# phylo42/IPK

Hardware: AMD Instinct MI355X
Metric: scored phylo-k-mers/sec (higher is better)
Workload: dtype f32

## Files before the change

ipk_amd/csrc/ipkgpu.hip:

```cpp
#include <cstring>
#include <hip/hip_runtime.h>
#include <rocprim/rocprim.hpp>

#include <algorithm>
#include <cmath>
#include <cstdarg>
#include <cstdio>
#include <cstring>
#include <new>
#include <string>
#include <type_traits>
#include <unordered_map>
#include <memory>
#include <vector>

#include "../../include/ipkgpu.h"
#include "dcla_device.hpp"
#include "kernels_score.hpp"
#include "kernels_quad.hpp"
#include "kernels_compact.hpp"
#include "kernels_keymajor.hpp"
#include "kernels_reduce_pipe.hpp"
#include "kernels_filter.hpp"
#include "kernels_dbfile.hpp"
// ... 53 lines not shown
struct ipkgpu_ctx {
    int device = 0;
    ipkgpu_comm* comm = nullptr;
    hipStream_t stream = nullptr;
    std::string err;
    int64_t workspace_bytes = 0;
    int64_t opt_variant = 0;
    int64_t opt_flags = 0;
    int64_t opt_kmc_pass = 0;
    int64_t opt_prefix_mats = 0;
    int64_t opt_wg_chunks2 = 0;
    int64_t opt_rounds = 0;
    int64_t opt_pool_limit = 0;
    int64_t opt_pool_chunks = 0;
    DevBuf table, best, ovfq, counts, offsets, goff, idx, branch, scan_sums, scan_boff, tmp_a, tmp_b, tmp_c;
    DevBuf pool, desc, gbcnt, gboff, gbcur, clist, gm, tile_next;
    DevBuf ptrs;
    DevBuf sp_bits, sp_pops, sp_rank, sp_c16;
    void* h_spill[2] = {nullptr, nullptr}; hipEvent_t ev_spill[2] = {nullptr, nullptr}; size_t h_spill_cap = 0;
    size_t held = 0, held_peak = 0;
    int64_t budget = 0;
    size_t refused_need = 0;
    DevBuf mask;
    bool mask_valid = false;
    uint64_t mask_words = 0;
    bool table_compressed = false;
    DevBuf rank, vaddr, ucnt, qpack, xstart, pcounts;
    DevBuf seq, pvals, pvaddr, mrank, cursnap;
    DevBuf cvals, coff, croom;
    bool comp_own_vals = false;
    std::vector<uint32_t> h_branch;
    uint32_t comp_nb = 0, comp_stride = 0, comp_tbl = 0;
    double pairs_per_window = 0;
    double acc_main_ms = 0, acc_reduce_ms = 0;
    double acc_count_ms = 0, acc_write_ms = 0, acc_km_ms = 0;
    const char* main_kernel = "";
    std::vector<std::pair<void*, size_t>> free_blocks;
    std::unordered_map<void*, size_t> live_blocks;
    size_t cached_bytes = 0, cache_limit = 0;
    void* small = nullptr;
    void* h_up = nullptr; size_t h_up_cap = 0; hipEvent_t up_done = nullptr; bool up_pending = false;
    unsigned long long emitted_host = 0; bool emitted_fetched = false;
    uint32_t* h_rb = nullptr;
    EventPool events;
    bool spec_skip_wait = false;
    uint64_t pool_want_min = 0;
    struct Pending {
        bool active = false;
        std::unique_ptr<Stopwatch> sw; int ev_a = -1, ev_b = -1, ev_c = -1, ev_d = -1;
        uint64_t cap = 0, max_chunks = 0, windows = 0; uint32_t gb = 0; bool pool_ovf_ok = false, use_quad = false;
    } pend;
    uint64_t last_entries = 0; uint32_t last_gb = 0;
    double t_write_total = 0, t_write_device = 0, t_write_file = 0;
    int num_cu = 256;
};

struct ipkgpu_result {
    ipkgpu_ctx* ctx = nullptr;
    std::vector<uint32_t> group_ids;
    std::vector<uint64_t> offsets;
    uint64_t emitted = 0;
    uint32_t* d_keys = nullptr;
    float* d_scores = nullptr;
    uint32_t* d_positions = nullptr;
    size_t cap = 0;
// ... 187 lines not shown
        *got = ctx->free_blocks[best].second;
        ctx->live_blocks[*out] = *got;
        ctx->cached_bytes -= *got;
        ctx->free_blocks.erase(ctx->free_blocks.begin() + best);
        return hipSuccess;
    }
    const hipError_t e = ctx_alloc(ctx, out, want_bytes);
    if (e == hipSuccess) *got = ctx->live_blocks[*out];
    return e;
}

static std::vector<DevBuf*> all_workspaces(ipkgpu_ctx* ctx)
{
    return {&ctx->table, &ctx->best, &ctx->ovfq, &ctx->counts, &ctx->offsets, &ctx->goff, &ctx->idx,
            &ctx->branch, &ctx->scan_sums, &ctx->scan_boff, &ctx->tmp_a, &ctx->tmp_b, &ctx->tmp_c,
            &ctx->pool, &ctx->desc, &ctx->gbcnt, &ctx->gboff, &ctx->gbcur, &ctx->clist, &ctx->gm, &ctx->tile_next, &ctx->mask,
            &ctx->rank, &ctx->vaddr, &ctx->ucnt, &ctx->qpack, &ctx->xstart, &ctx->pcounts, &ctx->ptrs,
            &ctx->cvals, &ctx->coff, &ctx->croom, &ctx->seq, &ctx->pvals, &ctx->pvaddr, &ctx->mrank, &ctx->cursnap,
            &ctx->sp_bits, &ctx->sp_pops, &ctx->sp_rank, &ctx->sp_c16};
}

extern "C" {

uint32_t ipkgpu_bits_per_symbol(uint32_t sigma) { return sigma == 4 ? 2u : sigma == 20 ? 5u : 0u; }
uint32_t ipkgpu_max_k(uint32_t sigma) { return sigma == 4 ? 14u : sigma == 20 ? 6u : 0u; }
uint32_t ipkgpu_max_k_keyrange(uint32_t sigma) { return sigma == 4 ? 16u : ipkgpu_max_k(sigma); }
size_t ipkgpu_kmer_batch(uint32_t key, size_t n_ranges) { return n_ranges ? key % n_ranges : 0; }

float ipkgpu_log_threshold(float omega, uint32_t sigma, uint32_t k)
{
    return log10f(powf(omega / (float)sigma, (float)k));
// ... 188 lines not shown
        constexpr int CAP = fast_cap<SIGMA, K>();
        constexpr uint32_t T = ipow(SIGMA, K);
        constexpr uint32_t NB = (T + TBL - 1) / TBL;
        constexpr int SNW = stream_nw<SIGMA, K>(), STW = stream_tw<SIGMA, K>();
        constexpr size_t lds = TileGeo<SIGMA, K, STW>::HEAD_BYTES + (size_t)SNW * stream_wave_scratch<SIGMA, K, CAP>() * 8 + (size_t)SNW * 2 * NB * SUB * 4;
        static_assert(lds <= 160 * 1024, "stream pass-1 LDS budget");
        auto kern = score_stream_kernel<SIGMA, K, CAP, STW, SNW, TBL>;
        if (lds > 64 * 1024)
            HIP_TRY(ctx, hipFuncSetAttribute(reinterpret_cast<const void*>(kern), hipFuncAttributeMaxDynamicSharedMemorySize, (int)lds));
        hipLaunchKernelGGL(kern, dim3(n_wg), dim3(SNW * 64), lds, ctx->stream, sp);
        HIP_TRY(ctx, hipGetLastError());
        return IPKGPU_OK;
    }
}

template <int SIGMA, int K>
int launch_stream_overflow(ipkgpu_ctx* ctx, const StreamParams& sp)
{
    constexpr uint32_t TBL = stream_tbl<SIGMA, K>();
    if constexpr (TBL == 0 || ipow(SIGMA, K - K / 2) <= (uint32_t)fast_cap<SIGMA, K>()) {
        (void)ctx; (void)sp;
        return IPKGPU_OK;
    } else {
        constexpr uint32_t NB = (uint32_t)((ipow(SIGMA, K) + TBL - 1) / TBL);
        constexpr size_t lds = TileGeo<SIGMA, K, 1>::HEAD_BYTES + (size_t)wave_scratch_entries<SIGMA, K, big_capf<SIGMA, K>()>() * 8 +
                               (size_t)OVF_NW * 2 * NB * SUB * 4;
        static_assert(lds + 64 <= 160 * 1024, "big-list (stream) LDS budget");
        auto kern = score_overflow_stream_kernel<SIGMA, K, TBL>;
        if (lds > 64 * 1024)
            HIP_TRY(ctx, hipFuncSetAttribute(reinterpret_cast<const void*>(kern), hipFuncAttributeMaxDynamicSharedMemorySize, (int)lds));
        const uint32_t per_cu = (uint32_t)std::max<size_t>(1, std::min<size_t>(32 / OVF_NW, (160 * 1024) / (lds + 64)));
        hipLaunchKernelGGL(kern, dim3(ctx->num_cu * per_cu), dim3(OVF_NW * 64), lds, ctx->stream, sp);
        HIP_TRY(ctx, hipGetLastError());
        return IPKGPU_OK;
    }
}

#ifndef IPK_RPIPE_DEFAULT
#define IPK_RPIPE_DEFAULT 1
#endif
#ifndef IPK_RPIPE_D
#define IPK_RPIPE_D 2
#endif
template <int SIGMA, int K>
int launch_stream_pass2(ipkgpu_ctx* ctx, uint32_t n_gb, uint64_t T, uint32_t* table, bool compress)
{
    constexpr uint32_t TBL = stream_tbl<SIGMA, K>();
// ... 274 lines not shown
{
    CompTable ct;
    ct.mask = ctx->mask.as<uint32_t>(); ct.rank = ctx->rank.as<uint32_t>(); ct.vaddr = ctx->vaddr.as<uint64_t>();
    ct.pool = ctx->comp_own_vals ? ctx->cvals.as<uint2>() : ctx->pool.as<uint2>();
    ct.off = ctx->comp_own_vals ? ctx->coff.as<uint64_t>() : ctx->gboff.as<uint64_t>(); ct.mask_words = ctx->mask_words;
    ct.NB = ctx->comp_nb; ct.stride = ctx->comp_stride; ct.TBL = ctx->comp_tbl;
    return ct;
}

}

namespace {

constexpr int IPKGPU_RETRY_SMALLER = 100;
constexpr int IPKGPU_RETRY_AGAIN = 101;
#ifndef IPK_OVF_POOL_RATIO
#define IPK_OVF_POOL_RATIO 500
#endif

enum class PassKind { tiles, stream, quad, xp };
struct Pass {
    PassKind kind = PassKind::tiles;
    bool positions = false;
    bool compress = false;
    bool seq = false;
    double slot_bytes() const { return positions ? 8.0 : kind == PassKind::xp && compress ? 0.3125 : 4.0; }
};

Pass choose_pass(int64_t variant, uint32_t sigma, uint32_t lead, bool positions, bool km_positions, const Geometry& g)
{
    Pass ps;
    ps.positions = positions;
    if (positions) return ps;
// ... 217 lines not shown
    pd.active = false;
    std::unique_ptr<Stopwatch> sw(pd.sw.release());
    const uint32_t n_ovf = ctx->h_rb[SMALL_OVF_COUNT / 4], pool_exhausted = ctx->h_rb[SMALL_POOL_OVF / 4];
    if (pool_exhausted) {
        if (pd.cap >= pd.max_chunks) {
            ctx->pool_want_min = 0;
            if (pd.gb > 1) return IPKGPU_RETRY_SMALLER;
            return fail(ctx, IPKGPU_ERR_NOMEM, "the pair pool of ONE branch group is exhausted at the device-memory limit");
        }
        ctx->pool_want_min = pd.cap * 2;
        return IPKGPU_RETRY_AGAIN;
    }
    ctx->pool_want_min = 0;
    memcpy(&ctx->emitted_host, ctx->h_rb + SMALL_EMITTED / 4, 8);
    ctx->emitted_fetched = true;
    ctx->spec_skip_wait = !(n_ovf > 0 && (uint64_t)n_ovf * IPK_OVF_POOL_RATIO >= pd.windows && pd.pool_ovf_ok);
    if (sw) { ctx->acc_main_ms += sw->ms(pd.ev_a, pd.ev_b); ctx->acc_reduce_ms += sw->ms(pd.ev_c, pd.ev_d); }
    return IPKGPU_OK;
}

int arm_capped(ipkgpu_ctx* ctx, uint32_t sigma, uint32_t k, ScoreParams& p)
{
    const bool capped_lists = sigma == 4 && k >= 13;
    p.big_ovf = capped_lists ? small_at(ctx, SMALL_BIG_OVF) : nullptr;
    if (capped_lists) HIP_TRY(ctx, hipMemsetAsync(p.big_ovf, 0, 4, ctx->stream));
    return IPKGPU_OK;
}

int check_capped(ipkgpu_ctx* ctx, uint32_t k, const ScoreParams& p)
{
    if (!p.big_ovf) return IPKGPU_OK;
// ... 162 lines not shown
    const uint64_t max_wg = std::max<uint64_t>(slots, expected_chunks * 2 / wg_chunks2 / ((uint64_t)SNW * NBK * SUB));
#ifndef IPK_ROUNDS
#define IPK_ROUNDS 8
#endif
    const uint64_t rounds = std::max<uint64_t>(1, std::min<uint64_t>(ctx->opt_rounds > 0 ? (uint64_t)ctx->opt_rounds : (uint64_t)IPK_ROUNDS, max_wg / slots));
    uint64_t S64 = std::max<uint64_t>(1, (slots * rounds) / gb);
    uint32_t S = (uint32_t)std::max<uint64_t>(1, std::min<uint64_t>(S64, s_tiles_per_mat));
    const uint32_t n_wg = gb * S;
    const uint64_t n_waves = (uint64_t)n_wg * SNW;
    const uint64_t n_gb = (uint64_t)gb * NBK;

    const size_t free_b = mem_free_bytes(ctx);
    uint64_t max_chunks = std::min<uint64_t>(0xFFFFFFF0ull, (uint64_t)(free_b + ctx->pool.cap + ctx->desc.cap) * 9 / 10 / (CH * 8 + 8));
    if (ctx->opt_pool_limit > 0) max_chunks = std::min<uint64_t>(max_chunks, (uint64_t)ctx->opt_pool_limit / (CH * 8 + 8));
    const double ppw = ctx->pairs_per_window > 0 ? ctx->pairs_per_window : 256.0;
    const uint64_t ovf_waves = (uint64_t)ctx->num_cu * 4 * OVF_NW;
    const uint64_t slack = 2 * (n_waves + ovf_waves) * NBK * SUB + (n_waves + ovf_waves) * ALLOC_BATCH + 1024;
    uint64_t want = (uint64_t)((double)windows * ppw * 1.25 / CH) + slack;
    {
        const uint64_t have = std::min<uint64_t>(std::max<uint64_t>(ctx->pool.cap / (CH * 8), 1) - 1, ctx->desc.cap / 8);
        const uint64_t need = (uint64_t)((double)windows * ppw * 1.1 / CH) + (n_waves + ovf_waves) * (NBK * SUB + ALLOC_BATCH) + 1024;
        if (have >= need) want = have;
    }
    want = std::max<uint64_t>(want, ctx->pool_want_min);
    for (int attempt = 0; attempt < 6; ++attempt) {
        uint64_t cap = std::min<uint64_t>(want, max_chunks);
        const bool forced = attempt == 0 && ctx->opt_pool_chunks > 0 && ctx->pool_want_min == 0;
        if (forced) cap = (uint64_t)ctx->opt_pool_chunks;
        else if (cap < n_waves * NBK * SUB) {
            if (gb > 1) return IPKGPU_RETRY_SMALLER;
            return fail(ctx, IPKGPU_ERR_NOMEM, "the pair pool of ONE branch group does not fit device memory");
// ... 1 lines not shown
        RC_TRY(ensure(ctx, ctx->pool, (cap + 1) * CH * 8));
        RC_TRY(ensure(ctx, ctx->desc, cap * 8));
        if (!forced) cap = std::min<uint64_t>(ctx->pool.cap / (CH * 8) - 1, ctx->desc.cap / 8);
        RC_TRY(ensure(ctx, ctx->gbcnt, 2 * n_gb * 4));
        uint32_t* const d_gbcur = ctx->gbcnt.as<uint32_t>() + n_gb;
        RC_TRY(ensure(ctx, ctx->gboff, (n_gb + 1) * 8));
        uint32_t* d_pool_next = small_at(ctx, SMALL_POOL_NEXT);
        uint32_t* d_pool_ovf = small_at(ctx, SMALL_POOL_OVF);
        const bool pre_ok = use_quad && n_waves * NBK + 1024 <= cap && !(ctx->opt_flags & 32);
        const uint32_t pre_chunks = pre_ok ? (uint32_t)(n_waves * NBK) : 0u;
        uint32_t* d_tile_next = nullptr;
        if (use_quad && !(ctx->opt_flags & 128) && ((uint64_t)nb * s_tiles_per_mat >= 4ull * gb * S || (ctx->opt_flags & 256))) {
            RC_TRY(ensure(ctx, ctx->tile_next, (size_t)gb * 4));
            d_tile_next = ctx->tile_next.as<uint32_t>();
        }
        hipLaunchKernelGGL(small_reset_kernel, dim3((std::max<uint32_t>(gb, SMALL_XP_TOO_BIG / 4) + 255) / 256), dim3(256), 0, ctx->stream,
                           reinterpret_cast<uint32_t*>(ctx->small), pre_chunks, d_tile_next, gb, S);
        HIP_TRY(ctx, hipGetLastError());
        HIP_TRY(ctx, hipMemsetAsync(ctx->desc.p, 0, cap * 8, ctx->stream));

        StreamParams sp;
        sp.logp = logp_dev; sp.best = ctx->best.as<float>();
        sp.gm_off = ctx->gm.as<uint32_t>(); sp.gm_list = ctx->gm.as<uint32_t>() + gb + 1;
        sp.sites = pl.sites; sp.nwin = pl.nwin; sp.tiles_per_mat = s_tiles_per_mat; sp.S = S;
        sp.eps = pl.eps;
        sp.pool = ctx->pool.as<uint2>(); sp.pool_cap = (uint32_t)cap; sp.pool_next = d_pool_next;
        sp.desc = ctx->desc.as<unsigned long long>(); sp.pool_ovf = d_pool_ovf;
        sp.emitted = p.emitted; sp.ovf_queue = p.ovf_queue; sp.ovf_count = p.ovf_count; sp.mat_slot = p.mat_slot;
        sp.flags = (uint32_t)(ctx->opt_flags);
        sp.pre_chunks = pre_chunks;
        sp.tile_next = d_tile_next;
        std::unique_ptr<Stopwatch> sw_own(new Stopwatch(ctx->stream, &ctx->events));
        Stopwatch& sw = *sw_own;
        const int ev_a = sw.mark();
        RC_TRY(pass1(sp, n_wg, false));
        const int ev_b = sw.mark();
        const bool spec = ctx->spec_skip_wait && !s_compress && !(ctx->opt_flags & 64);
        uint32_t n_ovf = 0;
        uint32_t h[2] = {0, 0};
        if (!spec) {
            HIP_TRY(ctx, hipMemcpyAsync(ctx->h_rb, ctx->small, SMALL_BYTES, hipMemcpyDeviceToHost, ctx->stream));
            HIP_TRY(ctx, hipStreamSynchronize(ctx->stream));
            n_ovf = ctx->h_rb[SMALL_OVF_COUNT / 4]; h[0] = ctx->h_rb[SMALL_POOL_NEXT / 4]; h[1] = ctx->h_rb[SMALL_POOL_OVF / 4];
        }
        const bool ovf_in_pool = n_ovf > 0 && ((uint64_t)n_ovf * IPK_OVF_POOL_RATIO >= windows || s_compress) && pool_ovf_ok;
        if (ovf_in_pool) {
            RC_TRY(ensure(ctx, ctx->tmp_a, (size_t)n_ovf * 8));
            RC_TRY(ensure(ctx, ctx->tmp_b, (size_t)n_ovf * 8));
            hipLaunchKernelGGL(ovf_group_keys_kernel, dim3((n_ovf + 255) / 256), dim3(256), 0, ctx->stream,
                               p.ovf_queue, n_ovf, p.mat_slot, ctx->tmp_a.as<unsigned long long>());
            HIP_TRY(ctx, hipGetLastError());
            size_t tmp_bytes = 0;
            HIP_TRY(ctx, rocprim::radix_sort_keys(nullptr, tmp_bytes, ctx->tmp_a.as<unsigned long long>(), ctx->tmp_b.as<unsigned long long>(),
                                                  (size_t)n_ovf, 0, 64, ctx->stream));
            RC_TRY(ensure(ctx, ctx->tmp_c, tmp_bytes));
            HIP_TRY(ctx, rocprim::radix_sort_keys(ctx->tmp_c.p, tmp_bytes, ctx->tmp_a.as<unsigned long long>(), ctx->tmp_b.as<unsigned long long>(),
                                                  (size_t)n_ovf, 0, 64, ctx->stream));
            StreamParams so = sp;
            so.ovf_queue = ctx->tmp_b.as<unsigned long long>();
            if (use_quad) so.emitted = small_at<unsigned long long>(ctx, SMALL_OVF_EMITTED);
            RC_TRY(with_sigma_k(ctx, pl.sigma, pl.k, [&](auto S_, auto K_) { return launch_stream_overflow<S_, K_>(ctx, so); }));
        }
        if (ovf_in_pool) {
            HIP_TRY(ctx, hipMemcpyAsync(ctx->h_rb, ctx->small, SMALL_BYTES, hipMemcpyDeviceToHost, ctx->stream));
            HIP_TRY(ctx, hipStreamSynchronize(ctx->stream));
            h[0] = ctx->h_rb[SMALL_POOL_NEXT / 4]; h[1] = ctx->h_rb[SMALL_POOL_OVF / 4];
        }
        if (h[1] != 0) {
            if (cap >= max_chunks) {
                if (gb > 1) return IPKGPU_RETRY_SMALLER;
                return fail(ctx, IPKGPU_ERR_NOMEM, "the pair pool of ONE branch group is exhausted at the device-memory limit");
            }
            want = std::max<uint64_t>(cap * 2, want);
            continue;
        }
        const uint32_t n_used = spec ? (uint32_t)cap : (uint32_t)std::min<uint64_t>(h[0], cap);
        const uint32_t* n_used_dev = spec ? d_pool_next : nullptr;
        HIP_TRY(ctx, hipMemsetAsync(ctx->gbcnt.p, 0, 2 * n_gb * 4, ctx->stream));
// ... 22 lines not shown
            RC_TRY(ensure(ctx, ctx->vaddr, (size_t)gb * (ctx->mask_words / 2) * 8));
            RC_TRY(ensure(ctx, ctx->ucnt, n_gb * 4));
        }
        if (n_used) {
            const uint64_t n_grid = spec ? std::min<uint64_t>(n_used, expected_chunks * 2 + n_waves * NBK + 4096) : n_used;
            hipLaunchKernelGGL(chunk_scatter_kernel, dim3((uint32_t)std::min<uint64_t>((n_grid + 255) / 256, 1u << 16)), dim3(256), 0, ctx->stream,
                               ctx->desc.as<unsigned long long>(), n_used, ctx->gboff.as<uint64_t>(), d_gbcur,
                               ctx->clist.as<uint2>(), n_used_dev);
            HIP_TRY(ctx, hipGetLastError());
        }
        const int ev_c = sw.mark();
        RC_TRY(with_sigma_k(ctx, pl.sigma, pl.k, [&](auto S_, auto K_) {
            return launch_stream_pass2<S_, K_>(ctx, (uint32_t)n_gb, pl.table_size, ctx->table.as<uint32_t>(), s_compress);
        }));
        const int ev_d = sw.mark();
        if ((spec || n_ovf > 0) && !ovf_in_pool)
            RC_TRY(with_sigma_k(ctx, pl.sigma, pl.k, [&](auto S_, auto K_) { return launch_overflow<S_, K_, false>(ctx, p); }));
        if (s_compress) {
            ctx->table_compressed = true; ctx->comp_own_vals = true;
            ctx->comp_nb = NBK; ctx->comp_stride = 1; ctx->comp_tbl = TBL;
        }
        ctx->mask_valid = true;
        ctx->main_kernel = use_quad ? "score_quad_kernel" : "score_stream_kernel";
        HIP_TRY(ctx, hipMemcpyAsync(ctx->h_rb, ctx->small, SMALL_BYTES, hipMemcpyDeviceToHost, ctx->stream));
        ipkgpu_ctx::Pending& pd = ctx->pend;
        pd.sw.reset(sw_own.release());
        pd.ev_a = ev_a; pd.ev_b = ev_b; pd.ev_c = ev_c; pd.ev_d = ev_d;
        pd.cap = cap; pd.max_chunks = max_chunks; pd.windows = windows; pd.gb = gb; pd.pool_ovf_ok = pool_ovf_ok; pd.use_quad = use_quad;
        pd.active = true;
        if (defer) return IPKGPU_OK;
        HIP_TRY(ctx, hipStreamSynchronize(ctx->stream));
        const int rcf = stream_batch_check(ctx);
        if (rcf == IPKGPU_RETRY_AGAIN) { want = std::max<uint64_t>(want, ctx->pool_want_min); continue; }
        return rcf;
    }
    return fail(ctx, IPKGPU_ERR_NOMEM, "pair pool could not be sized");
}

int score_batch_finish(ipkgpu_ctx* ctx, const Plan& pl, uint32_t g0, uint32_t gb, uint64_t* emitted_acc)
{
    if (ctx->pend.active) RC_TRY(stream_batch_check(ctx));
    unsigned long long e = ctx->emitted_host;
    if (!ctx->emitted_fetched) {
// ... 1325 lines not shown
        keys += f.head.n_keys; entries += f.head.n_entries;
    }
    return IPKGPU_OK;
}

}

extern "C" {

int ipkgpu_get_option(const ipkgpu_ctx* ctx, const char* name, int64_t* value)
{
    if (!ctx || !name || !value) return IPKGPU_ERR_INVALID;
    if (!strcmp(name, "workspace_bytes")) { *value = ctx->workspace_bytes; return IPKGPU_OK; }
    if (!strcmp(name, "device_budget_bytes")) { *value = ctx->budget; return IPKGPU_OK; }
    if (!strcmp(name, "last_refused_bytes")) { *value = (int64_t)ctx->refused_need; return IPKGPU_OK; }
    return IPKGPU_ERR_INVALID;
}

int ipkgpu_mem_stats(ipkgpu_ctx* ctx, uint64_t* held, uint64_t* held_peak, int reset_peak)
{
    if (!ctx) return IPKGPU_ERR_INVALID;
    if (held) *held = ctx->held;
    if (held_peak) *held_peak = ctx->held_peak;
    if (reset_peak) ctx->held_peak = ctx->held;
    return IPKGPU_OK;
}

int ipkgpu_parts_spill(ipkgpu_ctx* ctx, ipkgpu_parts* parts, const char* dir, uint32_t piece, uint64_t* bytes_written)
{
    if (!ctx) return IPKGPU_ERR_INVALID;
// ... 198 lines not shown
```

ipk_amd/csrc/kernels_quad.hpp:

```cpp
#pragma once
#include "kernels_score.hpp"

namespace ipkgpu {

struct QuadNode { int J, H, TH, OFF; uint32_t F, CMUL; };
struct QuadStep { int H, A, B; };

template <int SIGMA, int K>
struct QuadGeo {
    using D = HalvesDD<SIGMA, K>;
    static constexpr int HL = D::HL, HR = D::HR, LA = D::LA, LB = D::LB, RA = D::RA, RB = D::RB;
    static constexpr bool OK = SIGMA == 4 && D::OK && LA >= 2 && LA <= 3 && LB >= 2 && LB <= 3 && RA >= 2 && RA <= 3 && RB >= 2 && RB <= 3;
    static constexpr uint32_t FLA = D::FLA, FLB = D::FLB, FRA = D::FRA, FRB = D::FRB;
    static constexpr uint32_t mulR = ipow(SIGMA, K - K / 2);
    static constexpr uint32_t CW = FLA + FLB + FRA + FRB;
    static constexpr int th_n(int h) { return h == 2 ? 3 : 5; }
    static constexpr int TH0 = 2, TH1 = TH0 + th_n(LA), TH2 = TH1 + th_n(LB), TH3 = TH2 + th_n(RA);
    static constexpr int TH_F = TH3 + th_n(RB);
    static constexpr int PADW = 1;
    static constexpr QuadNode node(int n)
    {
        return n == 0 ? QuadNode{0, LA, TH0, 0, FLA, 1u}
             : n == 1 ? QuadNode{LA, LB, TH1, (int)FLA, FLB, mulR}
             : n == 2 ? QuadNode{HL, RA, TH2, (int)(FLA + FLB), FRA, 1u}
// ... 430 lines not shown
                    const bool p0 = v0 && c0, p1 = v1 && c1;
                    const uint64_t h0 = ballot64(v0) & ballot64(c0), h1 = ballot64(v1) & ballot64(c1);
                    if (p0) lp[mbcnt(h0)] = make_uint2(a0.x * (Q::FLB * mulR) + b0.x, __float_as_uint(s0));
                    if (p1) rp[mbcnt(h1)] = make_uint2(a1.x * Q::FRB + b1.x, __float_as_uint(s1));
                    nL = (uint32_t)__popcll(h0); nR = (uint32_t)__popcll(h1);
                } else {
                    if (!keep_l)
                        nL = (uint32_t)__builtin_amdgcn_readfirstlane((int)join_to_list(la + ia, min(sla, nla - ia), lb, nlb, eps_l, Q::FLB * mulR, lp, CAPL));
                    if constexpr (SLICE) {
                        if (nL == LIST_OVERFLOW) { sla = SAFE_L; continue; }
                    }
                    nR = nL == LIST_OVERFLOW || nL == 0 ? nL : (uint32_t)__builtin_amdgcn_readfirstlane((int)join_to_list(ra + ir, min(sra, nra - ir), rb, nrb, eps_r, Q::FRB, rp, CAPR));
                    if constexpr (SLICE) {
                        if (nR == LIST_OVERFLOW) { sra = SAFE_R; keep_l = true; continue; }
                    } else if (nL == LIST_OVERFLOW || nR == LIST_OVERFLOW) {
                        if (lane == 0) {
                            const uint32_t qi = atomicAdd(p.ovf_count, 1u);
                            p.ovf_queue[qi] = ((unsigned long long)mat << 32) | (unsigned long long)(t0 + w);
                        }
                        __builtin_amdgcn_wave_barrier();
                        break;
                    }
                }
                if (nL != 0 && nR != 0) {
                wave_lds_sync();
                if (p.flags & 4u) emitted += nL + nR;
                else
                if constexpr (ROWLANE) {
                    constexpr uint32_t CB = 64;
                    static_assert(CB <= CH, "row-per-lane join: a run must fit a chunk");
                    for (uint32_t ib = 0; ib < nL; ib += 64) {
                        const uint2 a = lp[ib + lane];
                        const bool rv = ib + lane < nL;
                        const float ay = rv ? __uint_as_float(a.y) : -__builtin_inff();
// ... 178 lines not shown
```

ipk_amd/csrc/kernels_score.hpp:

```cpp
#pragma once
#include <type_traits>
#include "dcla_device.hpp"

namespace ipkgpu {


template <int SIGMA, int M>
__global__ __launch_bounds__(256) void prefix_max_kernel(const float* __restrict__ logp, uint32_t n_mats, uint32_t sites,
                                                         float* __restrict__ best)
{
    constexpr int CH = 2048 / M;
    constexpr int ROW = CH + 4;
    static_assert(M == 1 || M == 2 || M == 4 || M == 8, "matrices per workgroup");
    __shared__ __align__(16) float cmbuf[2][M][ROW];
    const uint32_t mat0 = blockIdx.x * M;
    const uint32_t mv = min((uint32_t)M, n_mats - mat0);
    const bool chain = threadIdx.x < mv;
    const uint32_t my = mat0 + (chain ? threadIdx.x : 0u);
    float* b = best + (size_t)my * (sites + 1);
    if (chain) b[0] = 0.0f;
    float carry = 0.0f;
    auto maxima = [&](uint32_t c0, float (*cmw)[ROW], uint32_t t0, uint32_t nt) {
        const uint32_t n = min((uint32_t)CH, sites - c0);
        for (uint32_t mm = 0; mm < mv; ++mm) {
// ... 311 lines not shown
    uint32_t sites, nwin, tiles_per_mat, S;
    float eps;
    uint2* pool;
    uint32_t pool_cap;
    uint32_t* pool_next;
    unsigned long long* desc;
    uint32_t* pool_ovf;
    unsigned long long* emitted;
    unsigned long long* ovf_queue;
    uint32_t* ovf_count;
    const uint32_t* mat_slot;
    uint32_t flags;
    uint32_t pre_chunks;
    uint32_t* tile_next = nullptr;
    uint32_t* big_ovf = nullptr;
};

__device__ __constant__ uint32_t RCP16[65] = {
    0, 65536, 32768, 21846, 16384, 13108, 10923, 9363, 8192, 7282, 6554, 5958, 5462, 5042, 4682, 4370, 4096,
    3856, 3641, 3450, 3277, 3121, 2979, 2850, 2731, 2622, 2521, 2428, 2341, 2260, 2185, 2115, 2048,
    1986, 1928, 1873, 1821, 1772, 1725, 1681, 1639, 1599, 1561, 1525, 1490, 1457, 1425, 1395, 1366,
    1338, 1311, 1286, 1261, 1237, 1214, 1192, 1171, 1150, 1130, 1111, 1093, 1075, 1058, 1041, 1024};

template <int SIGMA, int K>
struct HalvesDD {
    static constexpr int HL = K / 2, HR = K - K / 2;
    static constexpr int LA = HL / 2, LB = HL - LA, RA = HR / 2, RB = HR - RA;
    static constexpr bool OK = ipow(SIGMA, HL) > 64 && ipow(SIGMA, LB) <= 64 && ipow(SIGMA, RB) <= 64;
    static constexpr uint32_t FLA = ipow(SIGMA, LA), FLB = ipow(SIGMA, LB), FRA = ipow(SIGMA, RA), FRB = ipow(SIGMA, RB);
};
template <int SIGMA, int K, int CAP>
// ... 175 lines not shown
            const uint32_t n4 = ncol * (SIGMA / 4);
            for (uint32_t i = threadIdx.x; i < n4; i += NW * 64) dst[i] = src[i];
            const float* bsrc = p.best + (size_t)mat * (p.sites + 1) + t0;
            for (uint32_t i = threadIdx.x; i <= ncol; i += NW * 64) best[i] = bsrc[i];
        }
        __syncthreads();
        for (uint32_t w = wave; w < nw; w += NW) {
            WinCtx c{cols, best, w};
            const uint2 *L, *R;
            uint32_t nL, nR;
            static_assert(!Geo<SIGMA, K, CAP>::DIRECT, "stream variant needs k with sigma^k > 64");
            bool ok;
            if constexpr (HalvesDD<SIGMA, K>::OK) ok = build_halves_dd<SIGMA, K, CAP>(c, p.eps, scratch, L, nL, R, nR);
            else ok = build_halves<SIGMA, K, CAP>(c, p.eps, scratch, L, nL, R, nR);
            if (!ok) {
                if (lane == 0) {
                    const uint32_t qi = atomicAdd(p.ovf_count, 1u);
                    p.ovf_queue[qi] = ((unsigned long long)mat << 32) | (unsigned long long)(t0 + w);
                }
                continue;
            }
            if (nL == 0 || nR == 0) continue;
            if (p.flags & 4u) { emitted += nL + nR; continue; }
            uint32_t cnt = 0;
            if (nR < 64) {
                const uint32_t total = nL * nR;
                const uint32_t M = RCP16[nR];
                const uint32_t q64 = (64u * M) >> 16, r64 = 64u - q64 * nR;
                uint32_t bi = 0, bj = 0;
                for (uint32_t base = 0; base < total; base += 128) {
                    uint32_t bi1 = bi + q64, bj1 = bj + r64;
                    if (bj1 >= nR) { bj1 -= nR; ++bi1; }
                    const uint32_t ta = bj + lane, tb = bj1 + lane;
                    const uint32_t qa = (ta * M) >> 16, qb = (tb * M) >> 16;
// ... 41 lines not shown

template <int SIGMA, int K, uint32_t TBL>
__global__ __launch_bounds__(OVF_NW * 64) void score_overflow_stream_kernel(StreamParams p)
{
    extern __shared__ __align__(16) unsigned char smem[];
    constexpr uint32_t CH = chunk_pairs<TBL>();
    constexpr int CAPF = big_capf<SIGMA, K>();
    constexpr uint32_t T = ipow(SIGMA, K);
    constexpr uint32_t NB = (T + TBL - 1) / TBL;
    using TG = TileGeo<SIGMA, K, 1>;
    __shared__ uint32_t sh_n[2];
    float* cols = reinterpret_cast<float*>(smem);
    float* best = cols + TG::COLS_F;
    uint2* scratch = reinterpret_cast<uint2*>(smem + TG::HEAD_BYTES);
    uint32_t* state_all = reinterpret_cast<uint32_t*>(scratch + wave_scratch_entries<SIGMA, K, CAPF>());
    const uint32_t n = *p.ovf_count;
    const uint32_t lane = lane_id(), wave = threadIdx.x >> 6;
    uint32_t* cbase = state_all + (size_t)wave * 2 * NB * SUB;
    uint32_t* cfill = cbase + NB * SUB;
    for (uint32_t b = lane; b < NB * SUB; b += 64) { cbase[b] = CHUNK_NONE; cfill[b] = CH; }
    Appender<TBL, NB> app{p, cbase, cfill, 0u};
    bool have_group = false;
    unsigned long long emitted = 0;
    constexpr uint32_t mulR = ipow(SIGMA, K - K / 2);
    auto close_chunks = [&]() {
        wave_lds_sync();
        for (uint32_t b = lane; b < NB * SUB; b += 64) {
            const uint32_t id = cbase[b];
            if (id != CHUNK_NONE) p.desc[id] = ((unsigned long long)(app.g * NB + b / SUB) << 32) | (unsigned long long)min(cfill[b], CH);
            cbase[b] = CHUNK_NONE; cfill[b] = CH;
        }
        wave_lds_sync();
    };
    const uint32_t per = (n + gridDim.x - 1) / gridDim.x;
    const uint32_t q_lo = min(n, blockIdx.x * per), q_hi = min(n, q_lo + per);
    for (uint32_t q = q_lo; q < q_hi; ++q) {
        const unsigned long long e = p.ovf_queue[q];
        const uint32_t g = (uint32_t)(e >> 42), mat = (uint32_t)(e >> 21) & 0x1FFFFFu, start = (uint32_t)e & 0x1FFFFFu;
        if (have_group && g != app.g) close_chunks();
        app.g = g; have_group = true;
        __syncthreads();
        const float* src = p.logp + ((size_t)mat * p.sites + start) * SIGMA;
        for (uint32_t i = threadIdx.x; i < K * SIGMA; i += OVF_NW * 64) cols[i] = src[i];
        const float* bsrc = p.best + (size_t)mat * (p.sites + 1) + start;
        for (uint32_t i = threadIdx.x; i <= K; i += OVF_NW * 64) best[i] = bsrc[i];
        __syncthreads();
        const uint2 *L = scratch, *R = scratch + Geo<SIGMA, K / 2, CAPF>::CAPH;
        if (wave == 0) {
            WinCtx c{cols, best, 0};
            uint32_t nL = 0, nR = 0;
            const bool fits = build_halves<SIGMA, K, CAPF>(c, p.eps, scratch, L, nL, R, nR);
            if (!fits) { nL = 0; nR = 0; if (lane == 0 && p.big_ovf) atomicOr(p.big_ovf, 1u); }
            if (lane == 0) { sh_n[0] = nL; sh_n[1] = nR; }
        }
        __syncthreads();
// ... 5 lines not shown
            for (uint32_t jb = 0; jb < nR; jb += 128) {
                const uint32_t ja = jb + lane, jc = jb + 64 + lane;
                const bool va = ja < nR, vb = jc < nR;
                uint2 b0 = make_uint2(0, 0), b1 = b0;
                if (va) b0 = R[ja];
                if (vb) b1 = R[jc];
                const float s0 = __uint_as_float(a.y) + __uint_as_float(b0.y);
                const float s1 = __uint_as_float(a.y) + __uint_as_float(b1.y);
                const bool p0 = va && (s0 > p.eps), p1 = vb && (s1 > p.eps);
                cnt += (uint32_t)__popcll(__ballot(p0)) + (uint32_t)__popcll(__ballot(p1));
                app.append2(p0, a.x * mulR + b0.x, __float_as_uint(s0), p1, a.x * mulR + b1.x, __float_as_uint(s1));
            }
        }
        emitted += cnt;
    }
    if (have_group) close_chunks();
    if (lane == 0 && emitted) atomicAdd(p.emitted, emitted);
}

__global__ __launch_bounds__(256) void ovf_group_keys_kernel(const unsigned long long* __restrict__ queue, uint32_t n,
                                                             const uint32_t* __restrict__ mat_slot,
                                                             unsigned long long* __restrict__ out)
{
    const uint32_t i = blockIdx.x * 256 + threadIdx.x;
    if (i >= n) return;
    const unsigned long long e = queue[i];
    const uint32_t mat = (uint32_t)(e >> 32), start = (uint32_t)e;
    out[i] = ((unsigned long long)mat_slot[mat] << 42) | ((unsigned long long)mat << 21) | (unsigned long long)start;
}

__global__ __launch_bounds__(256) void chunk_hist_kernel(const unsigned long long* __restrict__ desc, uint32_t n,
                                                         uint32_t* __restrict__ cnt, unsigned long long* __restrict__ pairs,
                                                         uint32_t* __restrict__ gb_pairs ,
                                                         const uint32_t* __restrict__ n_dev = nullptr)
{
    __shared__ unsigned long long wsum[4];
    unsigned long long c = 0;
    if (n_dev) n = min(n, *n_dev);
    for (uint32_t i = blockIdx.x * 256 + threadIdx.x; i < n; i += gridDim.x * 256) {
        const unsigned long long d = desc[i];
        if ((uint32_t)d != 0u) {
            atomicAdd(&cnt[(uint32_t)(d >> 32)], 1u);
            if (gb_pairs) atomicAdd(&gb_pairs[(uint32_t)(d >> 32)], (uint32_t)d);
// ... 22 lines not shown
        list[off[gb] + atomicAdd(&cur[gb], 1u)] = make_uint2(i, (uint32_t)d);
    }
}

constexpr uint32_t SMALL_EMITTED = 0;
constexpr uint32_t SMALL_OVF_COUNT = 16;
constexpr uint32_t SMALL_POOL_NEXT = 32;
constexpr uint32_t SMALL_POOL_OVF = 36;
constexpr uint32_t SMALL_BIG_OVF = 44;
constexpr uint32_t SMALL_OVF_EMITTED = 48;
constexpr uint32_t SMALL_XP_TOO_BIG = 56;
constexpr uint32_t SMALL_REC_BIG = 60;
constexpr uint32_t SMALL_BYTES = 64;

__global__ void small_reset_kernel(uint32_t* __restrict__ small, uint32_t pre_chunks, uint32_t* __restrict__ tile_next, uint32_t n_groups,
                                   uint32_t first_tile)
{
    const uint32_t i = blockIdx.x * blockDim.x + threadIdx.x;
    if (i < SMALL_XP_TOO_BIG / 4) small[i] = i == SMALL_POOL_NEXT / 4 ? pre_chunks : 0u;
    if (tile_next && i < n_groups) tile_next[i] = first_tile;
}

__device__ __forceinline__ void store_slice_mask(const uint32_t* tab, uint32_t nslots, uint32_t* mask_words, uint32_t nthreads)
{
    const uint32_t lane = lane_id(), wave = threadIdx.x >> 6, nwv = nthreads >> 6;
    const uint32_t nblk = (nslots + 63) / 64;
    const uint32_t bpw = (nblk + nwv - 1) / nwv;
    const uint32_t b_lo = min(nblk, wave * bpw), b_hi = min(nblk, b_lo + bpw);
    for (uint32_t b0 = b_lo; b0 < b_hi; b0 += 64) {
        const uint32_t nb = min(64u, b_hi - b0);
        uint64_t mine = 0;
#pragma unroll 4
        for (uint32_t j = 0; j < nb; ++j) {
            const uint32_t c = (b0 + j) * 64;
            const uint32_t v = (c + lane < nslots) ? tab[c + lane] : 0u;
// ... 777 lines not shown
```

Baseline: 132.9 billion.

## Bucket overflow windows per group on device and launch overflow pass speculatively

Overflowing windows are now queued directly into per-group slots, with the group index computed from blockIdx and read through kernarg loads. This replaces the global queue, the key-building kernel and the rocprim radix sort. The overflow kernel always launches right after pass 1 with a fixed grid of groups times workgroups-per-group, so the host no longer reads the overflow count back and synchronizes before deciding. The cost is that the queue is sized per group from gm_off*nwin, and the overflow grid launches even when no window overflows. It also adds a last_biglist_windows stat.

```diff
diff --git a/ipk_amd/csrc/ipkgpu.hip b/ipk_amd/csrc/ipkgpu.hip
--- a/ipk_amd/csrc/ipkgpu.hip
+++ b/ipk_amd/csrc/ipkgpu.hip
@@ -91,7 +91,7 @@
     int64_t opt_pool_limit = 0;
     int64_t opt_pool_chunks = 0;
     DevBuf table, best, ovfq, counts, offsets, goff, idx, branch, scan_sums, scan_boff, tmp_a, tmp_b, tmp_c;
-    DevBuf pool, desc, gbcnt, gboff, gbcur, clist, gm, tile_next;
+    DevBuf pool, desc, gbcnt, gboff, gbcur, clist, gm, tile_next, ovf_cnt;
     DevBuf ptrs;
     DevBuf sp_bits, sp_pops, sp_rank, sp_c16;
     void* h_spill[2] = {nullptr, nullptr}; hipEvent_t ev_spill[2] = {nullptr, nullptr}; size_t h_spill_cap = 0;
@@ -121,11 +121,12 @@
     uint32_t* h_rb = nullptr;
     EventPool events;
     bool spec_skip_wait = false;
+    uint32_t last_biglist_windows = 0;
     uint64_t pool_want_min = 0;
     struct Pending {
         bool active = false;
         std::unique_ptr<Stopwatch> sw; int ev_a = -1, ev_b = -1, ev_c = -1, ev_d = -1;
-        uint64_t cap = 0, max_chunks = 0, windows = 0; uint32_t gb = 0; bool pool_ovf_ok = false, use_quad = false;
+        uint64_t cap = 0, max_chunks = 0; uint32_t gb = 0; bool use_quad = false;
     } pend;
     uint64_t last_entries = 0; uint32_t last_gb = 0;
     double t_write_total = 0, t_write_device = 0, t_write_file = 0;
@@ -343,7 +344,7 @@
 {
     return {&ctx->table, &ctx->best, &ctx->ovfq, &ctx->counts, &ctx->offsets, &ctx->goff, &ctx->idx,
             &ctx->branch, &ctx->scan_sums, &ctx->scan_boff, &ctx->tmp_a, &ctx->tmp_b, &ctx->tmp_c,
-            &ctx->pool, &ctx->desc, &ctx->gbcnt, &ctx->gboff, &ctx->gbcur, &ctx->clist, &ctx->gm, &ctx->tile_next, &ctx->mask,
+            &ctx->pool, &ctx->desc, &ctx->gbcnt, &ctx->gboff, &ctx->gbcur, &ctx->clist, &ctx->gm, &ctx->tile_next, &ctx->ovf_cnt, &ctx->mask,
             &ctx->rank, &ctx->vaddr, &ctx->ucnt, &ctx->qpack, &ctx->xstart, &ctx->pcounts, &ctx->ptrs,
             &ctx->cvals, &ctx->coff, &ctx->croom, &ctx->seq, &ctx->pvals, &ctx->pvaddr, &ctx->mrank, &ctx->cursnap,
             &ctx->sp_bits, &ctx->sp_pops, &ctx->sp_rank, &ctx->sp_c16};
@@ -562,12 +563,18 @@
     }
 }
 
+constexpr uint32_t OVF_WG_MAX = 4;
+inline uint32_t ovf_wg_per_group(uint32_t num_cu, uint32_t gb)
+{
+    return std::max<uint32_t>(1, std::min<uint32_t>(OVF_WG_MAX, (2 * num_cu + gb - 1) / std::max<uint32_t>(gb, 1)));
+}
+
 template <int SIGMA, int K>
-int launch_stream_overflow(ipkgpu_ctx* ctx, const StreamParams& sp)
+int launch_stream_overflow(ipkgpu_ctx* ctx, const StreamParams& sp, uint32_t gb)
 {
     constexpr uint32_t TBL = stream_tbl<SIGMA, K>();
     if constexpr (TBL == 0 || ipow(SIGMA, K - K / 2) <= (uint32_t)fast_cap<SIGMA, K>()) {
-        (void)ctx; (void)sp;
+        (void)ctx; (void)sp; (void)gb;
         return IPKGPU_OK;
     } else {
         constexpr uint32_t NB = (uint32_t)((ipow(SIGMA, K) + TBL - 1) / TBL);
@@ -577,8 +584,8 @@
         auto kern = score_overflow_stream_kernel<SIGMA, K, TBL>;
         if (lds > 64 * 1024)
             HIP_TRY(ctx, hipFuncSetAttribute(reinterpret_cast<const void*>(kern), hipFuncAttributeMaxDynamicSharedMemorySize, (int)lds));
-        const uint32_t per_cu = (uint32_t)std::max<size_t>(1, std::min<size_t>(32 / OVF_NW, (160 * 1024) / (lds + 64)));
-        hipLaunchKernelGGL(kern, dim3(ctx->num_cu * per_cu), dim3(OVF_NW * 64), lds, ctx->stream, sp);
+        if ((uint64_t)gb * sp.S > 0x7fffffffull) return fail(ctx, IPKGPU_ERR_INVALID, "batch too large for one launch");
+        hipLaunchKernelGGL(kern, dim3(gb * sp.S), dim3(OVF_NW * 64), lds, ctx->stream, sp);
         HIP_TRY(ctx, hipGetLastError());
         return IPKGPU_OK;
     }
@@ -883,9 +890,6 @@
 
 constexpr int IPKGPU_RETRY_SMALLER = 100;
 constexpr int IPKGPU_RETRY_AGAIN = 101;
-#ifndef IPK_OVF_POOL_RATIO
-#define IPK_OVF_POOL_RATIO 500
-#endif
 
 enum class PassKind { tiles, stream, quad, xp };
 struct Pass {
@@ -1133,7 +1137,8 @@
     ctx->pool_want_min = 0;
     memcpy(&ctx->emitted_host, ctx->h_rb + SMALL_EMITTED / 4, 8);
     ctx->emitted_fetched = true;
-    ctx->spec_skip_wait = !(n_ovf > 0 && (uint64_t)n_ovf * IPK_OVF_POOL_RATIO >= pd.windows && pd.pool_ovf_ok);
+    ctx->spec_skip_wait = true;
+    ctx->last_biglist_windows = n_ovf;
     if (sw) { ctx->acc_main_ms += sw->ms(pd.ev_a, pd.ev_b); ctx->acc_reduce_ms += sw->ms(pd.ev_c, pd.ev_d); }
     return IPKGPU_OK;
 }
@@ -1326,7 +1331,8 @@
     uint64_t max_chunks = std::min<uint64_t>(0xFFFFFFF0ull, (uint64_t)(free_b + ctx->pool.cap + ctx->desc.cap) * 9 / 10 / (CH * 8 + 8));
     if (ctx->opt_pool_limit > 0) max_chunks = std::min<uint64_t>(max_chunks, (uint64_t)ctx->opt_pool_limit / (CH * 8 + 8));
     const double ppw = ctx->pairs_per_window > 0 ? ctx->pairs_per_window : 256.0;
-    const uint64_t ovf_waves = (uint64_t)ctx->num_cu * 4 * OVF_NW;
+    const uint32_t OVF_W = ovf_wg_per_group((uint32_t)ctx->num_cu, gb);
+    const uint64_t ovf_waves = pool_ovf_ok ? (uint64_t)gb * OVF_W * OVF_NW : 0;
     const uint64_t slack = 2 * (n_waves + ovf_waves) * NBK * SUB + (n_waves + ovf_waves) * ALLOC_BATCH + 1024;
     uint64_t want = (uint64_t)((double)windows * ppw * 1.25 / CH) + slack;
     {
@@ -1358,8 +1364,13 @@
             RC_TRY(ensure(ctx, ctx->tile_next, (size_t)gb * 4));
             d_tile_next = ctx->tile_next.as<uint32_t>();
         }
+        uint32_t* d_ovf_cnt = nullptr;
+        if (pool_ovf_ok) {
+            RC_TRY(ensure(ctx, ctx->ovf_cnt, (size_t)gb * 4));
+            d_ovf_cnt = ctx->ovf_cnt.as<uint32_t>();
+        }
         hipLaunchKernelGGL(small_reset_kernel, dim3((std::max<uint32_t>(gb, SMALL_XP_TOO_BIG / 4) + 255) / 256), dim3(256), 0, ctx->stream,
-                           reinterpret_cast<uint32_t*>(ctx->small), pre_chunks, d_tile_next, gb, S);
+                           reinterpret_cast<uint32_t*>(ctx->small), pre_chunks, d_tile_next, gb, S, d_ovf_cnt);
         HIP_TRY(ctx, hipGetLastError());
         HIP_TRY(ctx, hipMemsetAsync(ctx->desc.p, 0, cap * 8, ctx->stream));
 
@@ -1374,38 +1385,21 @@
         sp.flags = (uint32_t)(ctx->opt_flags);
         sp.pre_chunks = pre_chunks;
         sp.tile_next = d_tile_next;
+        sp.ovf_cnt = d_ovf_cnt;
         std::unique_ptr<Stopwatch> sw_own(new Stopwatch(ctx->stream, &ctx->events));
         Stopwatch& sw = *sw_own;
         const int ev_a = sw.mark();
         RC_TRY(pass1(sp, n_wg, false));
         const int ev_b = sw.mark();
+        if (pool_ovf_ok) {
+            StreamParams so = sp;
+            so.S = OVF_W;
+            if (use_quad) so.emitted = small_at<unsigned long long>(ctx, SMALL_OVF_EMITTED);
+            RC_TRY(with_sigma_k(ctx, pl.sigma, pl.k, [&](auto S_, auto K_) { return launch_stream_overflow<S_, K_>(ctx, so, gb); }));
+        }
         const bool spec = ctx->spec_skip_wait && !s_compress && !(ctx->opt_flags & 64);
-        uint32_t n_ovf = 0;
         uint32_t h[2] = {0, 0};
         if (!spec) {
-            HIP_TRY(ctx, hipMemcpyAsync(ctx->h_rb, ctx->small, SMALL_BYTES, hipMemcpyDeviceToHost, ctx->stream));
-            HIP_TRY(ctx, hipStreamSynchronize(ctx->stream));
-            n_ovf = ctx->h_rb[SMALL_OVF_COUNT / 4]; h[0] = ctx->h_rb[SMALL_POOL_NEXT / 4]; h[1] = ctx->h_rb[SMALL_POOL_OVF / 4];
-        }
-        const bool ovf_in_pool = n_ovf > 0 && ((uint64_t)n_ovf * IPK_OVF_POOL_RATIO >= windows || s_compress) && pool_ovf_ok;
-        if (ovf_in_pool) {
-            RC_TRY(ensure(ctx, ctx->tmp_a, (size_t)n_ovf * 8));
-            RC_TRY(ensure(ctx, ctx->tmp_b, (size_t)n_ovf * 8));
-            hipLaunchKernelGGL(ovf_group_keys_kernel, dim3((n_ovf + 255) / 256), dim3(256), 0, ctx->stream,
-                               p.ovf_queue, n_ovf, p.mat_slot, ctx->tmp_a.as<unsigned long long>());
-            HIP_TRY(ctx, hipGetLastError());
-            size_t tmp_bytes = 0;
-            HIP_TRY(ctx, rocprim::radix_sort_keys(nullptr, tmp_bytes, ctx->tmp_a.as<unsigned long long>(), ctx->tmp_b.as<unsigned long long>(),
-                                                  (size_t)n_ovf, 0, 64, ctx->stream));
-            RC_TRY(ensure(ctx, ctx->tmp_c, tmp_bytes));
-            HIP_TRY(ctx, rocprim::radix_sort_keys(ctx->tmp_c.p, tmp_bytes, ctx->tmp_a.as<unsigned long long>(), ctx->tmp_b.as<unsigned long long>(),
-                                                  (size_t)n_ovf, 0, 64, ctx->stream));
-            StreamParams so = sp;
-            so.ovf_queue = ctx->tmp_b.as<unsigned long long>();
-            if (use_quad) so.emitted = small_at<unsigned long long>(ctx, SMALL_OVF_EMITTED);
-            RC_TRY(with_sigma_k(ctx, pl.sigma, pl.k, [&](auto S_, auto K_) { return launch_stream_overflow<S_, K_>(ctx, so); }));
-        }
-        if (ovf_in_pool) {
             HIP_TRY(ctx, hipMemcpyAsync(ctx->h_rb, ctx->small, SMALL_BYTES, hipMemcpyDeviceToHost, ctx->stream));
             HIP_TRY(ctx, hipStreamSynchronize(ctx->stream));
             h[0] = ctx->h_rb[SMALL_POOL_NEXT / 4]; h[1] = ctx->h_rb[SMALL_POOL_OVF / 4];
@@ -1458,7 +1452,7 @@
             return launch_stream_pass2<S_, K_>(ctx, (uint32_t)n_gb, pl.table_size, ctx->table.as<uint32_t>(), s_compress);
         }));
         const int ev_d = sw.mark();
-        if ((spec || n_ovf > 0) && !ovf_in_pool)
+        if (!pool_ovf_ok)
             RC_TRY(with_sigma_k(ctx, pl.sigma, pl.k, [&](auto S_, auto K_) { return launch_overflow<S_, K_, false>(ctx, p); }));
         if (s_compress) {
             ctx->table_compressed = true; ctx->comp_own_vals = true;
@@ -1470,7 +1464,7 @@
         ipkgpu_ctx::Pending& pd = ctx->pend;
         pd.sw.reset(sw_own.release());
         pd.ev_a = ev_a; pd.ev_b = ev_b; pd.ev_c = ev_c; pd.ev_d = ev_d;
-        pd.cap = cap; pd.max_chunks = max_chunks; pd.windows = windows; pd.gb = gb; pd.pool_ovf_ok = pool_ovf_ok; pd.use_quad = use_quad;
+        pd.cap = cap; pd.max_chunks = max_chunks; pd.gb = gb; pd.use_quad = use_quad;
         pd.active = true;
         if (defer) return IPKGPU_OK;
         HIP_TRY(ctx, hipStreamSynchronize(ctx->stream));
@@ -2826,6 +2820,7 @@
     if (!strcmp(name, "workspace_bytes")) { *value = ctx->workspace_bytes; return IPKGPU_OK; }
     if (!strcmp(name, "device_budget_bytes")) { *value = ctx->budget; return IPKGPU_OK; }
     if (!strcmp(name, "last_refused_bytes")) { *value = (int64_t)ctx->refused_need; return IPKGPU_OK; }
+    if (!strcmp(name, "last_biglist_windows")) { *value = (int64_t)ctx->last_biglist_windows; return IPKGPU_OK; }
     return IPKGPU_ERR_INVALID;
 }
 
diff --git a/ipk_amd/csrc/kernels_quad.hpp b/ipk_amd/csrc/kernels_quad.hpp
--- a/ipk_amd/csrc/kernels_quad.hpp
+++ b/ipk_amd/csrc/kernels_quad.hpp
@@ -468,10 +468,7 @@
                     if constexpr (SLICE) {
                         if (nR == LIST_OVERFLOW) { sra = SAFE_R; keep_l = true; continue; }
                     } else if (nL == LIST_OVERFLOW || nR == LIST_OVERFLOW) {
-                        if (lane == 0) {
-                            const uint32_t qi = atomicAdd(p.ovf_count, 1u);
-                            p.ovf_queue[qi] = ((unsigned long long)mat << 32) | (unsigned long long)(t0 + w);
-                        }
+                        if (lane == 0) queue_big_window(p, mat, t0 + w);
                         __builtin_amdgcn_wave_barrier();
                         break;
                     }
diff --git a/ipk_amd/csrc/kernels_score.hpp b/ipk_amd/csrc/kernels_score.hpp
--- a/ipk_amd/csrc/kernels_score.hpp
+++ b/ipk_amd/csrc/kernels_score.hpp
@@ -349,7 +349,34 @@
     uint32_t pre_chunks;
     uint32_t* tile_next = nullptr;
     uint32_t* big_ovf = nullptr;
+    uint32_t* ovf_cnt = nullptr;
 };
+
+typedef const __attribute__((address_space(4))) unsigned char* karg_ptr;
+template <class T> __device__ __forceinline__ T karg_load(karg_ptr ka, size_t off)
+{
+    return *reinterpret_cast<const __attribute__((address_space(4))) T*>(ka + off);
+}
+__device__ __forceinline__ void queue_big_window(const StreamParams& p, uint32_t mat, uint32_t start)
+{
+    karg_ptr ka = (karg_ptr)__builtin_amdgcn_kernarg_segment_ptr();
+    (void)p;
+    asm volatile("" : "+s"(ka));
+    uint32_t* const cnt = karg_load<uint32_t*>(ka, offsetof(StreamParams, ovf_cnt));
+    uint32_t* const total = karg_load<uint32_t*>(ka, offsetof(StreamParams, ovf_count));
+    unsigned long long* const queue = karg_load<unsigned long long*>(ka, offsetof(StreamParams, ovf_queue));
+    if (cnt) {
+        const uint32_t g = blockIdx.x / karg_load<uint32_t>(ka, offsetof(StreamParams, S));
+        const uint32_t m0 = karg_load<const uint32_t*>(ka, offsetof(StreamParams, gm_off))[g];
+        const uint32_t qi = atomicAdd(&cnt[g], 1u);
+        queue[(size_t)m0 * karg_load<uint32_t>(ka, offsetof(StreamParams, nwin)) + qi] =
+            ((unsigned long long)g << 42) | ((unsigned long long)mat << 21) | (unsigned long long)start;
+        atomicAdd(total, 1u);
+    } else {
+        const uint32_t qi = atomicAdd(total, 1u);
+        queue[qi] = ((unsigned long long)mat << 32) | (unsigned long long)start;
+    }
+}
 
 __device__ __constant__ uint32_t RCP16[65] = {
     0, 65536, 32768, 21846, 16384, 13108, 10923, 9363, 8192, 7282, 6554, 5958, 5462, 5042, 4682, 4370, 4096,
@@ -555,10 +582,7 @@
             if constexpr (HalvesDD<SIGMA, K>::OK) ok = build_halves_dd<SIGMA, K, CAP>(c, p.eps, scratch, L, nL, R, nR);
             else ok = build_halves<SIGMA, K, CAP>(c, p.eps, scratch, L, nL, R, nR);
             if (!ok) {
-                if (lane == 0) {
-                    const uint32_t qi = atomicAdd(p.ovf_count, 1u);
-                    p.ovf_queue[qi] = ((unsigned long long)mat << 32) | (unsigned long long)(t0 + w);
-                }
+                if (lane == 0) queue_big_window(p, mat, t0 + w);
                 continue;
             }
             if (nL == 0 || nR == 0) continue;
@@ -630,31 +654,21 @@
     float* best = cols + TG::COLS_F;
     uint2* scratch = reinterpret_cast<uint2*>(smem + TG::HEAD_BYTES);
     uint32_t* state_all = reinterpret_cast<uint32_t*>(scratch + wave_scratch_entries<SIGMA, K, CAPF>());
-    const uint32_t n = *p.ovf_count;
+    const uint32_t g = blockIdx.x / p.S, seg = blockIdx.x - g * p.S;
+    const uint32_t m0 = p.gm_off[g];
+    const uint32_t n = min(p.ovf_cnt[g], (p.gm_off[g + 1] - m0) * p.nwin);
+    if (seg >= n) return;
+    const unsigned long long* queue = p.ovf_queue + (size_t)m0 * p.nwin;
     const uint32_t lane = lane_id(), wave = threadIdx.x >> 6;
     uint32_t* cbase = state_all + (size_t)wave * 2 * NB * SUB;
     uint32_t* cfill = cbase + NB * SUB;
     for (uint32_t b = lane; b < NB * SUB; b += 64) { cbase[b] = CHUNK_NONE; cfill[b] = CH; }
-    Appender<TBL, NB> app{p, cbase, cfill, 0u};
-    bool have_group = false;
+    Appender<TBL, NB> app{p, cbase, cfill, g};
     unsigned long long emitted = 0;
     constexpr uint32_t mulR = ipow(SIGMA, K - K / 2);
-    auto close_chunks = [&]() {
-        wave_lds_sync();
-        for (uint32_t b = lane; b < NB * SUB; b += 64) {
-            const uint32_t id = cbase[b];
-            if (id != CHUNK_NONE) p.desc[id] = ((unsigned long long)(app.g * NB + b / SUB) << 32) | (unsigned long long)min(cfill[b], CH);
-            cbase[b] = CHUNK_NONE; cfill[b] = CH;
-        }
-        wave_lds_sync();
-    };
-    const uint32_t per = (n + gridDim.x - 1) / gridDim.x;
-    const uint32_t q_lo = min(n, blockIdx.x * per), q_hi = min(n, q_lo + per);
-    for (uint32_t q = q_lo; q < q_hi; ++q) {
-        const unsigned long long e = p.ovf_queue[q];
-        const uint32_t g = (uint32_t)(e >> 42), mat = (uint32_t)(e >> 21) & 0x1FFFFFu, start = (uint32_t)e & 0x1FFFFFu;
-        if (have_group && g != app.g) close_chunks();
-        app.g = g; have_group = true;
+    for (uint32_t q = seg; q < n; q += p.S) {
+        const unsigned long long e = queue[q];
+        const uint32_t mat = (uint32_t)(e >> 21) & 0x1FFFFFu, start = (uint32_t)e & 0x1FFFFFu;
         __syncthreads();
         const float* src = p.logp + ((size_t)mat * p.sites + start) * SIGMA;
         for (uint32_t i = threadIdx.x; i < K * SIGMA; i += OVF_NW * 64) cols[i] = src[i];
@@ -690,19 +704,12 @@
         }
         emitted += cnt;
     }
-    if (have_group) close_chunks();
+    wave_lds_sync();
+    for (uint32_t b = lane; b < NB * SUB; b += 64) {
+        const uint32_t id = cbase[b];
+        if (id != CHUNK_NONE) p.desc[id] = ((unsigned long long)(g * NB + b / SUB) << 32) | (unsigned long long)min(cfill[b], CH);
+    }
     if (lane == 0 && emitted) atomicAdd(p.emitted, emitted);
-}
-
-__global__ __launch_bounds__(256) void ovf_group_keys_kernel(const unsigned long long* __restrict__ queue, uint32_t n,
-                                                             const uint32_t* __restrict__ mat_slot,
-                                                             unsigned long long* __restrict__ out)
-{
-    const uint32_t i = blockIdx.x * 256 + threadIdx.x;
-    if (i >= n) return;
-    const unsigned long long e = queue[i];
-    const uint32_t mat = (uint32_t)(e >> 32), start = (uint32_t)e;
-    out[i] = ((unsigned long long)mat_slot[mat] << 42) | ((unsigned long long)mat << 21) | (unsigned long long)start;
 }
 
 __global__ __launch_bounds__(256) void chunk_hist_kernel(const unsigned long long* __restrict__ desc, uint32_t n,
@@ -755,11 +762,12 @@
 constexpr uint32_t SMALL_BYTES = 64;
 
 __global__ void small_reset_kernel(uint32_t* __restrict__ small, uint32_t pre_chunks, uint32_t* __restrict__ tile_next, uint32_t n_groups,
-                                   uint32_t first_tile)
+                                   uint32_t first_tile, uint32_t* __restrict__ ovf_cnt)
 {
     const uint32_t i = blockIdx.x * blockDim.x + threadIdx.x;
     if (i < SMALL_XP_TOO_BIG / 4) small[i] = i == SMALL_POOL_NEXT / 4 ? pre_chunks : 0u;
     if (tile_next && i < n_groups) tile_next[i] = first_tile;
+    if (ovf_cnt && i < n_groups) ovf_cnt[i] = 0u;
 }
 
 __device__ __forceinline__ void store_slice_mask(const uint32_t* tab, uint32_t nslots, uint32_t* mask_words, uint32_t nthreads)
```

Result: slower. 129.3 billion (-2.7%).
